# globc/mrAudio

Hardware: AMD Instinct MI355X
Metric: clips/s encode+fuse+score, 32-clip x 32-frame synthetic (higher is better)
Workload: dtype f16

## Files before the change

### include/mra.h

```cpp
#ifndef MRA_H_
#define MRA_H_

#include <stddef.h>
#include <stdint.h>

#ifdef __cplusplus
extern "C" {
#endif

#define MRA_OK 0
#define MRA_EINVAL (-1)
#define MRA_ESTATE (-2)
#define MRA_EHIP (-3)
#define MRA_ENOMEM (-4)
#define MRA_ENAME (-5)

#define MRA_F32 0
#define MRA_F16 1
#define MRA_BF16 2

typedef struct mra_qformer mra_qformer;

typedef struct mra_cfg {
  int32_t hidden;
// ... 230 lines not shown
int mra_debug_self_attention(const void* qkv, const int64_t* mask, int32_t dtype, int32_t items, int32_t S, int32_t heads, void* ctx, float* lse,
                             void* stream);
int mra_debug_ln_rows(const float* x, const int64_t* x_view, int32_t rows, int32_t H, const float* const* params, int32_t lane_rows, int32_t period,
                      int32_t split, float eps, float* y32, const int64_t* y32_view, void* y16, const int64_t* y16_view, int32_t dtype, void* stream);
int mra_debug_embed_ln(const int64_t* ids, int32_t items, int32_t L, int32_t Q, int32_t H, int32_t vocab, const float* query, int64_t query_item_stride,
                       const float* word, const float* pos, const float* gain, const float* bias, float eps, float* h32, void* h16, float* pre32,
                       int32_t dtype, void* stream);
int mra_debug_modality_ln(const void* x, int32_t x_dtype, const int64_t* item_index, int32_t items, int32_t tokens, int32_t E, const float* gain,
                          const float* bias, float eps, void* out, int32_t dtype, void* stream);
int mra_debug_softmax_rows(const float* S, int64_t ld_s, void* P, int64_t ld_p, int32_t rows, int32_t kv, int32_t kvp, float scale, int32_t dtype,
                           void* stream);
int mra_debug_fold_query(const void* x, const int64_t* x_view, size_t x_bytes, const void* w_q, size_t w_q_bytes, const float* b_q, size_t b_q_bytes,
                         const void* w_k, size_t w_k_bytes, void* q_prime, size_t q_prime_bytes, int32_t rows, int32_t H, int32_t E, int32_t Q,
                         int32_t heads, int32_t dtype, void* stream);
int64_t mra_debug_fold_query_launches(void);
int64_t mra_debug_fold_rowfactor_launches(void);
int mra_debug_fold_rowfactor(const float* stat_m, const float* stat_l, float* factors, int32_t rows, int32_t R, int32_t ntiles, void* P, int64_t ld_p,
                             int32_t tile_cols, int32_t kvp, int32_t* hist, void* stream);
int mra_debug_softmax_rescale(void* P, int64_t ld_p, const float* stat_m, const float* stat_l, int32_t rows, int32_t ntiles, int32_t tile_cols,
                              int32_t kvp, int32_t dtype, int32_t* hist, void* stream);
int mra_debug_transpose_pad(const void* src, void* dst, int32_t R, int32_t C, int32_t ld_d, int64_t src_bs, int64_t dst_bs, int32_t batch, int32_t dtype,
                            void* stream);
int mra_debug_split(int32_t kind, const float* src, const int64_t* src_view, int32_t rows, int32_t C, int32_t chunk, int32_t parts, void* dst,
                    int32_t dtype, void* stream);

int mra_debug_gemm_tn_group(int32_t njobs, const void* const* dY, const int64_t* y_views, const int64_t* y_block_stride, const void* const* X,
                            const int64_t* x_views, const int64_t* x_block_stride, float* const* dW, float* const* db, const int32_t* M,
                            const int32_t* N, const int32_t* K, const int32_t* ldw, const int32_t* accumulate, int32_t dtype, void* stream);
int mra_debug_ln_bwd(const void* const* ptrs_a, const int64_t* views_a, int32_t rows_a, float eps_a, const void* const* ptrs_b, const int64_t* views_b,
                     int32_t rows_b, float eps_b, int32_t H, int32_t dtype, void* stream);
// ... 46 lines not shown
```

### mraudio_amd/_lib.py

```python
from __future__ import annotations

import ctypes as C
import os

import torch

MRA_F32, MRA_F16, MRA_BF16 = 0, 1, 2
_ERR = {-1: "MRA_EINVAL", -2: "MRA_ESTATE", -3: "MRA_EHIP", -4: "MRA_ENOMEM", -5: "MRA_ENAME"}

LIB_NAME = "libmra_hip.so"
LIB_PATH = os.path.join(os.path.dirname(os.path.abspath(__file__)), LIB_NAME)


class mra_cfg(C.Structure):
    _fields_ = [
        ("hidden", C.c_int32), ("heads", C.c_int32), ("inter", C.c_int32), ("layers", C.c_int32),
        ("cross_freq", C.c_int32), ("enc_width", C.c_int32), ("n_query", C.c_int32), ("vocab", C.c_int32),
        ("max_pos", C.c_int32), ("ln_eps", C.c_float), ("enc_ln_eps", C.c_float), ("llm_hidden", C.c_int32),
        ("op_dtype", C.c_int32),
    ]


class mra_vit_cfg(C.Structure):
    _fields_ = [("dim", C.c_int32), ("heads", C.c_int32), ("mlp", C.c_int32), ("depth", C.c_int32), ("patch", C.c_int32),
# ... 165 lines not shown
                                          C.c_int32, C.c_int32, C.c_int32, C.c_void_p, C.c_void_p, C.c_void_p, C.c_void_p]),
    "mra_debug_beats_attention": (C.c_int, [C.c_void_p, C.c_int32, C.c_void_p, C.c_void_p, C.c_int32, C.c_int32, C.c_void_p, C.c_void_p]),
    "mra_debug_beats_posconv": (C.c_int, [C.c_void_p, C.c_void_p, C.c_int32, C.c_int32, C.c_void_p]),
    "mra_debug_self_attention": (C.c_int, [C.c_void_p, C.c_void_p, C.c_int32, C.c_int32, C.c_int32, C.c_int32, C.c_void_p, C.c_void_p, C.c_void_p]),
    "mra_debug_ln_rows": (C.c_int, [C.c_void_p, C.POINTER(C.c_int64), C.c_int32, C.c_int32, C.POINTER(C.c_void_p), C.c_int32, C.c_int32, C.c_int32,
                                    C.c_float, C.c_void_p, C.POINTER(C.c_int64), C.c_void_p, C.POINTER(C.c_int64), C.c_int32, C.c_void_p]),
    "mra_debug_embed_ln": (C.c_int, [C.c_void_p, C.c_int32, C.c_int32, C.c_int32, C.c_int32, C.c_int32, C.c_void_p, C.c_int64, C.c_void_p, C.c_void_p,
                                     C.c_void_p, C.c_void_p, C.c_float, C.c_void_p, C.c_void_p, C.c_void_p, C.c_int32, C.c_void_p]),
    "mra_debug_modality_ln": (C.c_int, [C.c_void_p, C.c_int32, C.c_void_p, C.c_int32, C.c_int32, C.c_int32, C.c_void_p, C.c_void_p, C.c_float,
                                        C.c_void_p, C.c_int32, C.c_void_p]),
    "mra_debug_softmax_rows": (C.c_int, [C.c_void_p, C.c_int64, C.c_void_p, C.c_int64, C.c_int32, C.c_int32, C.c_int32, C.c_float, C.c_int32,
                                         C.c_void_p]),
    "mra_debug_fold_query": (C.c_int, [C.c_void_p, C.c_void_p, C.c_size_t, C.c_void_p, C.c_size_t, C.c_void_p, C.c_size_t, C.c_void_p, C.c_size_t,
                                       C.c_void_p, C.c_size_t, C.c_int32, C.c_int32, C.c_int32, C.c_int32, C.c_int32, C.c_int32, C.c_void_p]),
    "mra_debug_fold_query_launches": (C.c_int64, []),
    "mra_debug_fold_rowfactor_launches": (C.c_int64, []),
    "mra_debug_fold_rowfactor": (C.c_int, [C.c_void_p, C.c_void_p, C.c_void_p, C.c_int32, C.c_int32, C.c_int32, C.c_void_p, C.c_int64, C.c_int32,
                                           C.c_int32, C.c_void_p, C.c_void_p]),
    "mra_debug_softmax_rescale": (C.c_int, [C.c_void_p, C.c_int64, C.c_void_p, C.c_void_p, C.c_int32, C.c_int32, C.c_int32, C.c_int32, C.c_int32,
                                            C.c_void_p, C.c_void_p]),
    "mra_debug_transpose_pad": (C.c_int, [C.c_void_p, C.c_void_p, C.c_int32, C.c_int32, C.c_int32, C.c_int64, C.c_int64, C.c_int32, C.c_int32,
                                          C.c_void_p]),
    "mra_debug_split": (C.c_int, [C.c_int32, C.c_void_p, C.POINTER(C.c_int64), C.c_int32, C.c_int32, C.c_int32, C.c_int32, C.c_void_p, C.c_int32,
                                  C.c_void_p]),
    "mra_debug_gemm_tn_group": (C.c_int, [C.c_int32, C.POINTER(C.c_void_p), C.POINTER(C.c_int64), C.POINTER(C.c_int64), C.POINTER(C.c_void_p),
                                          C.POINTER(C.c_int64), C.POINTER(C.c_int64), C.POINTER(C.c_void_p), C.POINTER(C.c_void_p), C.POINTER(C.c_int32),
                                          C.POINTER(C.c_int32), C.POINTER(C.c_int32), C.POINTER(C.c_int32), C.POINTER(C.c_int32), C.c_int32, C.c_void_p]),
    "mra_debug_ln_bwd": (C.c_int, [C.POINTER(C.c_void_p), C.POINTER(C.c_int64), C.c_int32, C.c_float, C.POINTER(C.c_void_p), C.POINTER(C.c_int64),
                                   C.c_int32, C.c_float, C.c_int32, C.c_int32, C.c_void_p]),
    "mra_debug_embed_bwd": (C.c_int, [C.c_void_p, C.c_void_p, C.c_int32, C.c_int32, C.c_int32, C.c_int32, C.c_int32, C.c_void_p, C.c_void_p, C.c_void_p,
# ... 84 lines not shown
```

### mraudio_amd/csrc/attention.hip

```cpp
#include "kernels.h"
#include "mra_common.h"

namespace mra {

namespace {

typedef int i32x4v __attribute__((ext_vector_type(4)));

constexpr int KVT = 32;
constexpr int TILE_B = KVT * 128;
constexpr int WAVE_LDS = 4 * TILE_B;
constexpr int OPAD = 68;
constexpr float LOG2E = 1.4426950408889634f;
constexpr int PART_STRIDE = 32 * 64 + 64;
constexpr int SH_TPS = 2;
constexpr int SH_STAGES = 3;
constexpr int SH_STAGE_B = SH_TPS * 2 * TILE_B;
constexpr int SH_PARK_B = (32 * OPAD + 64) * 4;
constexpr int SH_LDS = SH_STAGES * SH_STAGE_B > 4 * SH_PARK_B ? SH_STAGES * SH_STAGE_B : 4 * SH_PARK_B;

template <typename T, bool MASKED, int SPLITW>
__global__ void __launch_bounds__(256) attn_kernel(const AttnArgs a) {
  extern __shared__ __attribute__((aligned(16))) char smem[];
  const int tid = threadIdx.x;
  const int lane = tid & 63;
  const int wave = __builtin_amdgcn_readfirstlane(tid >> 6);
  const int qblocks = (a.q_rows + 31) >> 5;
  const int nunits = a.items * a.heads * qblocks;
  const int ntiles_all = (a.kv_len + KVT - 1) / KVT;

  int unit, gs;
  if (SPLITW == 1) {
    unit = blockIdx.x * 4 + wave;
    gs = 0;
  } else {
// ... 81 lines not shown
#pragma unroll
  for (int i = 0; i < 16; ++i) { ot[0][i] = 0.f; ot[1][i] = 0.f; }

  const int h4 = 4 * (lane >> 5);
  int buf = 0;
  if (tfirst < te) issue(0, tfirst);
  for (int t = tfirst; t < te; t += tstep) {
    const bool more = t + tstep < te;
    if (more) {
      issue(buf ^ 1, t + tstep);
      asm volatile("s_waitcnt vmcnt(8)" ::: "memory");
    } else {
      asm volatile("s_waitcnt vmcnt(0)" ::: "memory");
    }
    const char* kb = wl + buf * 2 * TILE_B;
    const char* vb = kb + TILE_B;

    f32x16 st;
#pragma unroll
    for (int i = 0; i < 16; ++i) st[i] = 0.f;
#pragma unroll
    for (int s = 0; s < 4; ++s) st = mfma32<T>(lds_read8<T>(kb + koff[s]), qf[s], st);

    const int tok0 = t * KVT;
    float mx = -INFINITY;
#pragma unroll
    for (int g4 = 0; g4 < 4; ++g4) {
      f32x4 madd;
      if (MASKED) {
        madd = *reinterpret_cast<const f32x4*>(wmask + tok0 + 8 * g4 + h4);
      }
#pragma unroll
      for (int e = 0; e < 4; ++e) {
        const int i = 4 * g4 + e;
        float y = st[i] * sl2;
        if (MASKED) {
          y += madd[e];
        } else {
          if (tok0 + 8 * g4 + h4 + e >= a.kv_len) y = -INFINITY;
        }
        st[i] = y;
        mx = fmaxf(mx, y);
      }
    }
    mx = fmaxf(mx, __shfl_xor(mx, 32, 64));
    const float m_new = fmaxf(m_run, mx);
    const float alpha = __builtin_amdgcn_exp2f(m_run - m_new);
    m_run = m_new;
    float psum = 0.f;
#pragma unroll
    for (int i = 0; i < 16; ++i) {
      const float p = __builtin_amdgcn_exp2f(st[i] - m_new);
      st[i] = p;
      psum += p;
    }
    l_run = l_run * alpha + psum;
#pragma unroll
    for (int i = 0; i < 16; ++i) { ot[0][i] *= alpha; ot[1][i] *= alpha; }

    typename Vec8<T>::type pf[2];
#pragma unroll
    for (int s = 0; s < 2; ++s)
#pragma unroll
      for (int j = 0; j < 8; ++j) pf[s][j] = from_f32<T>(st[8 * s + j]);

    {
      const unsigned vaddr0 = wl_lds + buf * 2 * TILE_B + TILE_B + vlane[0];
      const unsigned vaddr1 = wl_lds + buf * 2 * TILE_B + TILE_B + vlane[1];
      i16x4 r00, r01, r02, r03, r10, r11, r12, r13;
      asm volatile(
          "ds_read_b64_tr_b16 %0, %8\n\t"
          "ds_read_b64_tr_b16 %1, %8 offset:1024\n\t"
          "ds_read_b64_tr_b16 %2, %8 offset:2048\n\t"
          "ds_read_b64_tr_b16 %3, %8 offset:3072\n\t"
          "ds_read_b64_tr_b16 %4, %9\n\t"
          "ds_read_b64_tr_b16 %5, %9 offset:1024\n\t"
          "ds_read_b64_tr_b16 %6, %9 offset:2048\n\t"
          "ds_read_b64_tr_b16 %7, %9 offset:3072\n\t"
          "s_waitcnt lgkmcnt(0)"
          : "=&v"(r00), "=&v"(r01), "=&v"(r02), "=&v"(r03), "=&v"(r10), "=&v"(r11), "=&v"(r12), "=&v"(r13)
          : "v"(vaddr0), "v"(vaddr1)
          : "memory");
      auto cat = [](i16x4 lo, i16x4 hi) {
        i16x8 v8;
        v8[0] = lo[0]; v8[1] = lo[1]; v8[2] = lo[2]; v8[3] = lo[3];
        v8[4] = hi[0]; v8[5] = hi[1]; v8[6] = hi[2]; v8[7] = hi[3];
        return __builtin_bit_cast(typename Vec8<T>::type, v8);
      };
      ot[0] = mfma32<T>(cat(r00, r01), pf[0], ot[0]);
      ot[0] = mfma32<T>(cat(r02, r03), pf[1], ot[0]);
      ot[1] = mfma32<T>(cat(r10, r11), pf[0], ot[1]);
      ot[1] = mfma32<T>(cat(r12, r13), pf[1], ot[1]);
    }
    buf ^= 1;
  }

  const float l_tot = l_run + __shfl_xor(l_run, 32, 64);
  float* ow = reinterpret_cast<float*>(wl);
  float* mw = ow + 32 * OPAD;
  float* lw = mw + 32;
  {
    const int q = lane & 31;
#pragma unroll
    for (int mt = 0; mt < 2; ++mt)
#pragma unroll
      for (int g4 = 0; g4 < 4; ++g4) {
        f32x4 v = {ot[mt][4 * g4], ot[mt][4 * g4 + 1], ot[mt][4 * g4 + 2], ot[mt][4 * g4 + 3]};
        *reinterpret_cast<f32x4*>(ow + q * OPAD + 32 * mt + 8 * g4 + h4) = v;
// ... 63 lines not shown
    const f32x4 x1 = *reinterpret_cast<const f32x4*>(ps + q * 64 + 8 * dc + 4);
#pragma unroll
    for (int e = 0; e < 4; ++e) { o[e] += wgt * x0[e]; o[4 + e] += wgt * x1[e]; }
  }
  const int q0 = qb * 32;
  if (q0 + q >= a.q_rows) return;
  if (a.lse && dc == 0) a.lse[((long long)item * a.heads + head) * a.q_rows + q0 + q] = M + __builtin_amdgcn_logf(L);
  const float inv = 1.0f / L;
  typename Vec8<T>::type r;
#pragma unroll
  for (int e = 0; e < 8; ++e) r[e] = from_f32<T>(o[e] * inv);
  T* op = (T*)a.O + (long long)item * a.o_item_stride + (long long)(q0 + q) * a.o_ld + head * 64 + 8 * dc;
  *reinterpret_cast<typename Vec8<T>::type*>(op) = r;
}

template <typename T>
int launch_t(const AttnArgs& a, hipStream_t stream) {
  const int qblocks = (a.q_rows + 31) >> 5;
  const int nunits = a.items * a.heads * qblocks;
  const int ntiles = (a.kv_len + KVT - 1) / KVT;
  const bool masked = a.mask != nullptr;
  const bool shared = ntiles >= 8 && !masked;
  size_t lds = 4 * WAVE_LDS + (masked ? (size_t)4 * ntiles * KVT * sizeof(float) : 0);
  if (lds > 160 * 1024) return -1;
  void (*kfn)(const AttnArgs);
  dim3 grid;
  if (shared) {
    kfn = attn_kernel<T, false, 4>;
    grid = dim3(nunits * a.nsplit);
  } else {
    if (a.nsplit != 1) return -1;
    kfn = masked ? attn_kernel<T, true, 1> : attn_kernel<T, false, 1>;
    grid = dim3((nunits + 3) / 4);
  }
  if (lds > 64 * 1024) {
    if (hipFuncSetAttribute((const void*)kfn, hipFuncAttributeMaxDynamicSharedMemorySize, (int)lds) != hipSuccess)
      return -3;
  }
  hipLaunchKernelGGL(kfn, grid, dim3(256), lds, stream, a);
  if (shared && a.nsplit > 1) {
    hipLaunchKernelGGL(attn_combine_kernel<T>, dim3(nunits), dim3(256), 0, stream, a);
  }
  return hipGetLastError() == hipSuccess ? 0 : -4;
}

template <typename T>
__global__ void __launch_bounds__(256) attn_shared_kernel(const AttnArgs a) {
  extern __shared__ __attribute__((aligned(16))) char smem[];
  const int tid = threadIdx.x;
  const int lane = tid & 63;
  const int wave = __builtin_amdgcn_readfirstlane(tid >> 6);
  const int groups = (a.kv_share + 3) >> 2;
  const int ntiles_all = (a.kv_len + KVT - 1) / KVT;
  const int nstages_all = (ntiles_all + SH_TPS - 1) / SH_TPS;

  int b = blockIdx.x;
  const int gs = b % a.nsplit; b /= a.nsplit;
  const int grp = b % groups; b /= groups;
  const int head = b % a.heads;
// ... 229 lines not shown
    if ((long long)nunits * s >= 1536) break;
  }
  return best;
}

int launch_attention(const AttnArgs& args, int op_dtype, hipStream_t stream) {
  AttnArgs a = args;
  if (a.kv_share < 1) a.kv_share = 1;
  if (a.items <= 0 || a.heads <= 0 || a.q_rows <= 0 || a.kv_len <= 0 || a.nsplit < 1) return -1;
  if (a.nsplit > 1 && !a.part) return -1;
  if ((a.q_ld | a.o_ld | a.k_ld | a.v_ld) & 7) return -1;
  if (a.items % a.kv_share) return -1;
  return op_dtype == OP_F16 ? launch_t<f16>(a, stream) : launch_t<bf16>(a, stream);
}

int attn_shared_pick_split(int kv_items, int kv_share, int heads, int kv_len) {
  const int units = kv_items * heads * ((kv_share + 3) / 4);
  const int ntiles = (kv_len + KVT - 1) / KVT;
  const int nstages = (ntiles + SH_TPS - 1) / SH_TPS;
  if (ntiles < 64) return 1;
  int best = 1;
  for (int s = 1; s <= 16; ++s) {
    if (nstages / s < 8) break;
    best = s;
    if ((long long)units * s >= 512) break;
  }
  return best;
}

int launch_attention_shared(const AttnArgs& args, int op_dtype, hipStream_t stream) {
// ... 10 lines not shown
```

### mraudio_amd/csrc/kernels.h

```cpp
#pragma once
#include <hip/hip_runtime.h>
#include <stdint.h>

namespace mra {

enum OpDtype { OP_F16 = 0, OP_BF16 = 1 };

enum GemmEpi {
  EPI_OP = 0,
  EPI_GELU_OP = 1,
  EPI_RES_F32 = 2,
  EPI_F32 = 3,
  EPI_KV = 4,
  EPI_GELU_BOTH = 6,
  EPI_GELU_BWD = 7,
  EPI_RES_OP = 8,
  EPI_RES_LN = 9,
  EPI_RES_F32_STAT = 10,
  EPI_RES_OP_STAT = 13,
  EPI_LNF_OP = 11,
  EPI_LNF_GELU_OP = 12,
  EPI_SOFTPART = 5,
};

// ... 248 lines not shown
  int k_ld, v_ld;
  const long long* mask;
  int mask_ld;
  int items, heads, q_rows, kv_len;
  float scale;
  int nsplit;
  float* part;
  float* lse;
  int kv_share = 1;
};
size_t attn_partial_bytes(int items, int heads, int q_rows, int nsplit);
int attn_pick_split(int items, int heads, int q_rows, int kv_len);
int launch_attention(const AttnArgs& a, int op_dtype, hipStream_t stream);
int attn_shared_pick_split(int kv_items, int kv_share, int heads, int kv_len);
int launch_attention_shared(const AttnArgs& a, int op_dtype, hipStream_t stream);

int launch_ln_rows(const float* x, RowView xv, int rows, int H, const float* gain, const float* bias, float eps,
                   float* y32, RowView y32v, void* y16, RowView y16v, int op_dtype, hipStream_t stream);
int launch_ln_rows2(const float* x, RowView xv, int rows, int H, const float* gain, const float* bias, const float* gain2,
                    const float* bias2, int period, int split, float eps, float* y32, RowView y32v, void* y16, RowView y16v,
                    int op_dtype, hipStream_t stream);
int launch_ln_rows4(const float* x, RowView xv, int rows, int H, const float* gain, const float* bias, const float* gain2, const float* bias2,
                    int lane_rows, const float* gain3, const float* bias3, const float* gain4, const float* bias4, int period, int split,
                    float eps, float* y32, RowView y32v, void* y16, RowView y16v, int op_dtype, hipStream_t stream);
int launch_modality_ln(const void* x, int x_dtype, const long long* item_index, int items, int tokens, int E,
                       const float* gain, const float* bias, float eps, void* out, int op_dtype, hipStream_t stream);
int launch_embed_ln(const long long* ids, int items, int L, int Q, int H, int vocab, const float* query,
                    long long query_item_stride, const float* word,
                    const float* pos, const float* gain, const float* bias, float eps, float* h32, void* h16,
                    float* pre32 , int op_dtype, hipStream_t stream);
// ... 22 lines not shown
```

### mraudio_amd/csrc/mra_abi.hip

```cpp
#include <cmath>
#include <cstdio>
#include <cstdlib>

#include "mra_handle.h"

using namespace mra;
using namespace mra_host;

namespace mra_host {
thread_local std::string g_err;
}

namespace {

size_t layout_params(mra_qformer* h, char* base) {
  const mra_cfg& c = h->cfg;
  const size_t H = c.hidden, I = c.inter, E = c.enc_width;
  Carver cv(base);
  size_t goff = 0;
  auto reg = [&](const std::string& name, void* p, int dtype, long long numel) {
    Param pr;
    pr.ptr = p;
    pr.dtype = dtype;
    pr.numel = numel;
// ... 580 lines not shown
  return per_item * items;
}

namespace {
int check_loaded(mra_qformer* h) {
  char names[256];
  const int miss = mra_qformer_missing(h, names, sizeof(names));
  int tolerated = 0;
  for (const char* opt : {"ln.weight", "ln.bias", "llm_proj.weight", "llm_proj.bias"}) {
    auto it = h->params.find(opt);
    if (it != h->params.end() && !it->second.loaded) ++tolerated;
  }
  return miss > tolerated ? fail(MRA_ESTATE, std::string("parameters not loaded: ") + names) : MRA_OK;
}

int run_lanes(Lane* lanes, int nl, const int64_t* input_ids, const int64_t* attention_mask, int N, int L, void* workspace, hipStream_t stream) {
  const mra_qformer* h = lanes[0].h;
  const mra_cfg& c = h->cfg;
  const bool pair = nl == 2;
  const int Q = c.n_query, S = Q + L, H = c.hidden, I = c.inter;
  const int op = h->op();
  long long* mask2 = nullptr;
  layout_lanes(lanes, nl, (char*)workspace, N, L, &mask2);
  const Work& w = lanes[0].w;
  const long long SH = (long long)S * H;
  const size_t esz = 2;

  const RowView all_rows = plain(N * S, H), all_lanes = plain(nl * N * S, H);
  const RowView q_view = items_view(SH, Q, H);
  const RowView t_view = items_view(SH, L > 0 ? L : 1, H);
  const RowView cls_view = items_view(SH, 1, H);
  const RowView qc_rows = plain(N * Q, H);
  const size_t t_off16 = (size_t)Q * H * esz;
  const size_t t_off32 = (size_t)Q * H;

  const bool ln_fuse = !pair && (h->chain_ring & 12) == 12 && H % 96 == 0 && H % 256 == 0 && H <= 1024;
  int rc;
  for (int l = 0; l < nl; ++l) {
    Lane& x = lanes[l];
    mra_qformer* hl = x.h;
    rc = launch_embed_ln((const long long*)input_ids, N, L, Q, H, hl->cfg.vocab, x.query, x.query_stride, hl->word, hl->pos, hl->embg, hl->embb,
                         c.ln_eps, x.w.hA32, x.w.hA16, nullptr, op, stream);
    if (rc) return chk(rc, "embed_ln");
    if (ln_fuse) HIP_TRY(hipMemsetAsync(w.lncnt, 0, w.lncnt_bytes, stream));
    if (x.plan.form != CrossPlan::KV_CACHE) {
      if (x.plan.form == CrossPlan::FOLD && !x.plan.kmajor) {
        const int E = hl->cfg.enc_width, kvp = fold_kvp(x.kv);
        rc = launch_transpose_pad(x.enc, x.w.encT, x.kv, E, kvp, (long long)x.kv * E, (long long)E * kvp, N, op, stream);
        if (rc) return chk(rc, "enc transpose");
      }
// ... 9 lines not shown
  }
  const long long* mask = (const long long*)attention_mask;
  if (pair && mask) {
    HIP_TRY(hipMemcpyAsync(mask2, mask, (size_t)N * S * 8, hipMemcpyDeviceToDevice, stream));
    HIP_TRY(hipMemcpyAsync(mask2 + (size_t)N * S, mask, (size_t)N * S * 8, hipMemcpyDeviceToDevice, stream));
    mask = mask2;
  }

  const bool want_text_last = lanes[0].out_full != nullptr;
  bool want_cls_last = false;
  for (int l = 0; l < nl; ++l) want_cls_last |= !want_text_last && lanes[l].out_cls;

  for (int i = 0; i < c.layers; ++i) {
    const LayerW* Lw[2] = {&lanes[0].h->layers[i], &lanes[nl - 1].h->layers[i]};
    const bool last = i == c.layers - 1;
    {
      GemmProb p[2] = {};
      for (int l = 0; l < nl; ++l) {
        p[l].A = lanes[l].w.hA16; p[l].a = all_rows;
        p[l].W = Lw[l]->wqkv; p[l].bias = Lw[l]->bqkv;
        p[l].C = lanes[l].w.qkv16; p[l].c = plain(N * S, 3 * H);
        p[l].M = N * S; p[l].N = 3 * H; p[l].K = H;
        p[l].tile_cfg = N * S >= 1024 ? GT_128 : GT_AUTO;
        if ((lanes[l].h->chain_ring & 1) && N * S >= 1024 && (3 * H) % 144 == 0) p[l].tile_cfg = GT_RING_144x128;
      }
      rc = launch_gemm(p, nl, EPI_OP, op, stream);
      if (rc) return chk(rc, "qkv gemm");
    }
    rc = launch_attention(self_attn_args(c, w.qkv16, w.ctx16, mask, nl * N, S), op, stream);
    if (rc) return chk(rc, "self attention");
    {
      GemmProb p[2] = {};
      for (int l = 0; l < nl; ++l) {
        p[l].A = lanes[l].w.ctx16; p[l].a = all_rows;
        p[l].W = Lw[l]->wo; p[l].bias = Lw[l]->bo;
        p[l].R = lanes[l].w.hA32; p[l].r = all_rows;
        p[l].C = lanes[l].w.pre32; p[l].c = all_rows;
        p[l].M = N * S; p[l].N = H; p[l].K = H;
        if ((lanes[l].h->chain_ring & 4) && N * S >= 1024 && H % 96 == 0) p[l].tile_cfg = GT_RING_96x64;
      }
      if (ln_fuse && p[0].tile_cfg == GT_RING_96x64) {
        p[0].ln_gain = Lw[0]->ln1g; p[0].ln_bias = Lw[0]->ln1b; p[0].ln_eps = c.ln_eps;
        p[0].ln_y32 = w.hB32; p[0].ln_y32v = all_rows; p[0].ln_y16 = w.hB16; p[0].ln_y16v = all_rows; p[0].ln_counter = w.lncnt;
        rc = launch_gemm(p, 1, EPI_RES_LN, op, stream);
        if (rc) return chk(rc, "attn out gemm + ln");
// ... 551 lines not shown
    if (value < 0 || value > 1000) return fail(MRA_EINVAL, "auto_split_pmax_milli is a threshold on p_max in [0, 1000] thousandths");
    h->auto_tau_milli = value;
    return MRA_OK;
  }
  if (key == "chain_ring") {
    if (value < 0 || value > 15) return fail(MRA_EINVAL, "chain_ring is a mask of bits 0-3");
    h->chain_ring = value;
    return MRA_OK;
  }
  if (key == "cross_fuse") {
    if (value < 0 || (value & ~7))
      return fail(MRA_EINVAL, "cross_fuse is a mask of 1 (query projection and Q' in one launch), 2 (row factors inside the P.enc launch) and 4 (context GEMM on the 64 x 64 tile)");
    h->cross_fuse = value;
    return MRA_OK;
  }
  if (key == "multi_core") {
    if (value < 0 || value > 1) return fail(MRA_EINVAL, "multi_core is 0 (attn_kernel with kv_share) or 1 (shared-stream core)");
    h->multi_core = value;
    return MRA_OK;
  }
  return fail(MRA_ENAME, "unknown option: " + key);
}

int mra_qformer_set_kv_done_event(mra_qformer* h, void* ev) {
  if (!h) return fail(MRA_EINVAL, "null handle");
  h->kv_done = reinterpret_cast<hipEvent_t>(ev);
  return MRA_OK;
}

size_t mra_kv_cache_bytes(mra_qformer* h, int32_t items, int32_t kv) {
// ... 789 lines not shown
  if (rows == 0) return MRA_OK;
  if (!x || !w_q || !w_k || !q_prime) return fail(MRA_EINVAL, "null argument");
  if (!dbg_aligned(x, 16) || !dbg_aligned(w_q, 16) || !dbg_aligned(w_k, 16) || !dbg_aligned(q_prime, 16) || !dbg_aligned(b_q, 16))
    return fail(MRA_EINVAL, "misaligned buffer");
  if (!dbg_fits(dbg_extent(xv, rows, H), 2, 0, x_bytes)) return fail(MRA_EINVAL, "x: the view and H leave x_bytes");
  if (!dbg_fits((u128)heads * 64 * (u128)H, 2, 0, w_q_bytes)) return fail(MRA_EINVAL, "w_q: heads * 64 rows of H leave w_q_bytes");
  if (b_q && !dbg_fits((u128)heads * 64, 4, 0, b_q_bytes)) return fail(MRA_EINVAL, "b_q: heads * 64 floats leave b_q_bytes");
  if (!dbg_fits((u128)heads * (u128)E * 64, 2, 0, w_k_bytes)) return fail(MRA_EINVAL, "w_k: heads blocks of [E][64] leave w_k_bytes");
  if (!dbg_fits((u128)rows * (u128)heads * (u128)E, 2, 0, q_prime_bytes)) return fail(MRA_EINVAL, "q_prime: rows * heads * E elements leave q_prime_bytes");
  return chk(launch_fold_query(x, xv, w_q, b_q, w_k, q_prime, rows, H, E, Q, heads, op, as_stream(stream)), "fold_query");
}

int64_t mra_debug_fold_query_launches(void) { return fold_query_launch_count(); }
int64_t mra_debug_fold_rowfactor_launches(void) { return fold_rowfactor_launch_count(); }

}
```

### mraudio_amd/csrc/mra_handle.h

```cpp
#pragma once
#include <hip/hip_runtime.h>

#include <algorithm>
#include <cstdlib>
#include <cstring>
#include <map>
#include <string>
#include <vector>

#include "../../include/mra.h"
#include "kernels.h"
#include "mra_common.h"

namespace mra_host {

using namespace mra;

extern thread_local std::string g_err;

inline int fail(int code, const std::string& msg) {
  g_err = msg;
  return code;
}

// ... 105 lines not shown
  float *encg = nullptr, *encb = nullptr;
  void* wkv = nullptr;
  float* bkv = nullptr;
  void* wllm = nullptr;
  float* bllm = nullptr;
  char* arena_f = nullptr;
  bool fold_stale = true;
  bool raw_features = true;
  bool inreg_rescale = true;
  int fold_tile = mra::GT_128;
  bool fold_stream = false;
  int cross_mode = 0;
  int chain_ring = 7;
  int train_ring = 4;
  int cross_fuse = 1;
  int multi_core = 1;
  int cross_precise = 0;
  float* wk32 = nullptr;
  char* arena_p = nullptr;
  bool precise_stale = true;
  bool cross_auto = false;
  bool auto_stale = true;
  int auto_resolved = -1;
  int auto_probes = 0;
  int auto_tau_milli = 500;
  int* auto_hist = nullptr;
  int* auto_hist_host = nullptr;
  std::vector<float> auto_median;
  hipEvent_t kv_done = nullptr;
  hipEvent_t kv_ev0 = nullptr, kv_ev1 = nullptr;
// ... 54 lines not shown
```

Measured before the change: 4942.

## Fuse QKV projection GEMM and self-attention into one kernel launch

```diff
diff --git a/include/mra.h b/include/mra.h
--- a/include/mra.h
+++ b/include/mra.h
@@ -268,6 +268,12 @@
                          const void* w_k, size_t w_k_bytes, void* q_prime, size_t q_prime_bytes, int32_t rows, int32_t H, int32_t E, int32_t Q,
                          int32_t heads, int32_t dtype, void* stream);
 int64_t mra_debug_fold_query_launches(void);
+int mra_debug_qkv_attention(const void* rows, const void* wqkv, const float* bqkv, const int64_t* mask, int32_t dtype, int32_t items, int32_t S,
+                            int32_t heads, void* ctx, void* stream);
+int64_t mra_debug_qkv_attention_launches(void);
+int64_t mra_debug_attention_launches(int32_t masked);
+int32_t mra_debug_self_fuse_plan(int32_t option, int32_t chain_ring, int32_t lanes, int32_t items, int32_t S, int32_t hidden, int32_t heads,
+                                 int32_t dtype, int32_t want_full);
 int64_t mra_debug_fold_rowfactor_launches(void);
 int mra_debug_fold_rowfactor(const float* stat_m, const float* stat_l, float* factors, int32_t rows, int32_t R, int32_t ntiles, void* P, int64_t ld_p,
                              int32_t tile_cols, int32_t kvp, int32_t* hist, void* stream);
diff --git a/mraudio_amd/_lib.py b/mraudio_amd/_lib.py
--- a/mraudio_amd/_lib.py
+++ b/mraudio_amd/_lib.py
@@ -203,6 +203,11 @@
     "mra_debug_fold_query": (C.c_int, [C.c_void_p, C.c_void_p, C.c_size_t, C.c_void_p, C.c_size_t, C.c_void_p, C.c_size_t, C.c_void_p, C.c_size_t,
                                        C.c_void_p, C.c_size_t, C.c_int32, C.c_int32, C.c_int32, C.c_int32, C.c_int32, C.c_int32, C.c_void_p]),
     "mra_debug_fold_query_launches": (C.c_int64, []),
+    "mra_debug_qkv_attention": (C.c_int, [C.c_void_p, C.c_void_p, C.c_void_p, C.c_void_p, C.c_int32, C.c_int32, C.c_int32, C.c_int32, C.c_void_p,
+                                          C.c_void_p]),
+    "mra_debug_qkv_attention_launches": (C.c_int64, []),
+    "mra_debug_attention_launches": (C.c_int64, [C.c_int32]),
+    "mra_debug_self_fuse_plan": (C.c_int32, [C.c_int32, C.c_int32, C.c_int32, C.c_int32, C.c_int32, C.c_int32, C.c_int32, C.c_int32, C.c_int32]),
     "mra_debug_fold_rowfactor_launches": (C.c_int64, []),
     "mra_debug_fold_rowfactor": (C.c_int, [C.c_void_p, C.c_void_p, C.c_void_p, C.c_int32, C.c_int32, C.c_int32, C.c_void_p, C.c_int64, C.c_int32,
                                            C.c_int32, C.c_void_p, C.c_void_p]),
diff --git a/mraudio_amd/csrc/attention.hip b/mraudio_amd/csrc/attention.hip
--- a/mraudio_amd/csrc/attention.hip
+++ b/mraudio_amd/csrc/attention.hip
@@ -1,3 +1,6 @@
+#include <atomic>
+#include <type_traits>
+
 #include "kernels.h"
 #include "mra_common.h"
 
@@ -19,6 +22,87 @@
 constexpr int SH_PARK_B = (32 * OPAD + 64) * 4;
 constexpr int SH_LDS = SH_STAGES * SH_STAGE_B > 4 * SH_PARK_B ? SH_STAGES * SH_STAGE_B : 4 * SH_PARK_B;
 
+template <typename T, bool MASKED>
+__device__ __forceinline__ void attn_tile_step(const char* kb, unsigned vtile, const int (&koff)[4], const unsigned (&vlane)[2],
+                                               const typename Vec8<T>::type (&qf)[4], const float* wm, int tok0, int kv_len, float sl2, int h4,
+                                               float& m_run, float& l_run, f32x16 (&ot)[2]) {
+  f32x16 st;
+#pragma unroll
+  for (int i = 0; i < 16; ++i) st[i] = 0.f;
+#pragma unroll
+  for (int s = 0; s < 4; ++s) st = mfma32<T>(lds_read8<T>(kb + koff[s]), qf[s], st);
+
+  float mx = -INFINITY;
+#pragma unroll
+  for (int g4 = 0; g4 < 4; ++g4) {
+    f32x4 madd;
+    if (MASKED) {
+      madd = *reinterpret_cast<const f32x4*>(wm + 8 * g4 + h4);
+    }
+#pragma unroll
+    for (int e = 0; e < 4; ++e) {
+      const int i = 4 * g4 + e;
+      float y = st[i] * sl2;
+      if (MASKED) {
+        y += madd[e];
+      } else {
+        if (tok0 + 8 * g4 + h4 + e >= kv_len) y = -INFINITY;
+      }
+      st[i] = y;
+      mx = fmaxf(mx, y);
+    }
+  }
+  mx = fmaxf(mx, __shfl_xor(mx, 32, 64));
+  const float m_new = fmaxf(m_run, mx);
+  const float alpha = __builtin_amdgcn_exp2f(m_run - m_new);
+  m_run = m_new;
+  float psum = 0.f;
+#pragma unroll
+  for (int i = 0; i < 16; ++i) {
+    const float p = __builtin_amdgcn_exp2f(st[i] - m_new);
+    st[i] = p;
+    psum += p;
+  }
+  l_run = l_run * alpha + psum;
+#pragma unroll
+  for (int i = 0; i < 16; ++i) { ot[0][i] *= alpha; ot[1][i] *= alpha; }
+
+  typename Vec8<T>::type pf[2];
+#pragma unroll
+  for (int s = 0; s < 2; ++s)
+#pragma unroll
+    for (int j = 0; j < 8; ++j) pf[s][j] = from_f32<T>(st[8 * s + j]);
+
+  {
+    const unsigned vaddr0 = vtile + vlane[0];
+    const unsigned vaddr1 = vtile + vlane[1];
+    i16x4 r00, r01, r02, r03, r10, r11, r12, r13;
+    asm volatile(
+        "ds_read_b64_tr_b16 %0, %8\n\t"
+        "ds_read_b64_tr_b16 %1, %8 offset:1024\n\t"
+        "ds_read_b64_tr_b16 %2, %8 offset:2048\n\t"
+        "ds_read_b64_tr_b16 %3, %8 offset:3072\n\t"
+        "ds_read_b64_tr_b16 %4, %9\n\t"
+        "ds_read_b64_tr_b16 %5, %9 offset:1024\n\t"
+        "ds_read_b64_tr_b16 %6, %9 offset:2048\n\t"
+        "ds_read_b64_tr_b16 %7, %9 offset:3072\n\t"
+        "s_waitcnt lgkmcnt(0)"
+        : "=&v"(r00), "=&v"(r01), "=&v"(r02), "=&v"(r03), "=&v"(r10), "=&v"(r11), "=&v"(r12), "=&v"(r13)
+        : "v"(vaddr0), "v"(vaddr1)
+        : "memory");
+    auto cat = [](i16x4 lo, i16x4 hi) {
+      i16x8 v8;
+      v8[0] = lo[0]; v8[1] = lo[1]; v8[2] = lo[2]; v8[3] = lo[3];
+      v8[4] = hi[0]; v8[5] = hi[1]; v8[6] = hi[2]; v8[7] = hi[3];
+      return __builtin_bit_cast(typename Vec8<T>::type, v8);
+    };
+    ot[0] = mfma32<T>(cat(r00, r01), pf[0], ot[0]);
+    ot[0] = mfma32<T>(cat(r02, r03), pf[1], ot[0]);
+    ot[1] = mfma32<T>(cat(r10, r11), pf[0], ot[1]);
+    ot[1] = mfma32<T>(cat(r12, r13), pf[1], ot[1]);
+  }
+}
+
 template <typename T, bool MASKED, int SPLITW>
 __global__ void __launch_bounds__(256) attn_kernel(const AttnArgs a) {
   extern __shared__ __attribute__((aligned(16))) char smem[];
@@ -130,84 +214,8 @@
       asm volatile("s_waitcnt vmcnt(0)" ::: "memory");
     }
     const char* kb = wl + buf * 2 * TILE_B;
-    const char* vb = kb + TILE_B;
-
-    f32x16 st;
-#pragma unroll
-    for (int i = 0; i < 16; ++i) st[i] = 0.f;
-#pragma unroll
-    for (int s = 0; s < 4; ++s) st = mfma32<T>(lds_read8<T>(kb + koff[s]), qf[s], st);
-
-    const int tok0 = t * KVT;
-    float mx = -INFINITY;
-#pragma unroll
-    for (int g4 = 0; g4 < 4; ++g4) {
-      f32x4 madd;
-      if (MASKED) {
-        madd = *reinterpret_cast<const f32x4*>(wmask + tok0 + 8 * g4 + h4);
-      }
-#pragma unroll
-      for (int e = 0; e < 4; ++e) {
-        const int i = 4 * g4 + e;
-        float y = st[i] * sl2;
-        if (MASKED) {
-          y += madd[e];
-        } else {
-          if (tok0 + 8 * g4 + h4 + e >= a.kv_len) y = -INFINITY;
-        }
-        st[i] = y;
-        mx = fmaxf(mx, y);
-      }
-    }
-    mx = fmaxf(mx, __shfl_xor(mx, 32, 64));
-    const float m_new = fmaxf(m_run, mx);
-    const float alpha = __builtin_amdgcn_exp2f(m_run - m_new);
-    m_run = m_new;
-    float psum = 0.f;
-#pragma unroll
-    for (int i = 0; i < 16; ++i) {
-      const float p = __builtin_amdgcn_exp2f(st[i] - m_new);
-      st[i] = p;
-      psum += p;
-    }
-    l_run = l_run * alpha + psum;
-#pragma unroll
-    for (int i = 0; i < 16; ++i) { ot[0][i] *= alpha; ot[1][i] *= alpha; }
-
-    typename Vec8<T>::type pf[2];
-#pragma unroll
-    for (int s = 0; s < 2; ++s)
-#pragma unroll
-      for (int j = 0; j < 8; ++j) pf[s][j] = from_f32<T>(st[8 * s + j]);
-
-    {
-      const unsigned vaddr0 = wl_lds + buf * 2 * TILE_B + TILE_B + vlane[0];
-      const unsigned vaddr1 = wl_lds + buf * 2 * TILE_B + TILE_B + vlane[1];
-      i16x4 r00, r01, r02, r03, r10, r11, r12, r13;
-      asm volatile(
-          "ds_read_b64_tr_b16 %0, %8\n\t"
-          "ds_read_b64_tr_b16 %1, %8 offset:1024\n\t"
-          "ds_read_b64_tr_b16 %2, %8 offset:2048\n\t"
-          "ds_read_b64_tr_b16 %3, %8 offset:3072\n\t"
-          "ds_read_b64_tr_b16 %4, %9\n\t"
-          "ds_read_b64_tr_b16 %5, %9 offset:1024\n\t"
-          "ds_read_b64_tr_b16 %6, %9 offset:2048\n\t"
-          "ds_read_b64_tr_b16 %7, %9 offset:3072\n\t"
-          "s_waitcnt lgkmcnt(0)"
-          : "=&v"(r00), "=&v"(r01), "=&v"(r02), "=&v"(r03), "=&v"(r10), "=&v"(r11), "=&v"(r12), "=&v"(r13)
-          : "v"(vaddr0), "v"(vaddr1)
-          : "memory");
-      auto cat = [](i16x4 lo, i16x4 hi) {
-        i16x8 v8;
-        v8[0] = lo[0]; v8[1] = lo[1]; v8[2] = lo[2]; v8[3] = lo[3];
-        v8[4] = hi[0]; v8[5] = hi[1]; v8[6] = hi[2]; v8[7] = hi[3];
-        return __builtin_bit_cast(typename Vec8<T>::type, v8);
-      };
-      ot[0] = mfma32<T>(cat(r00, r01), pf[0], ot[0]);
-      ot[0] = mfma32<T>(cat(r02, r03), pf[1], ot[0]);
-      ot[1] = mfma32<T>(cat(r10, r11), pf[0], ot[1]);
-      ot[1] = mfma32<T>(cat(r12, r13), pf[1], ot[1]);
-    }
+    attn_tile_step<T, MASKED>(kb, wl_lds + buf * 2 * TILE_B + TILE_B, koff, vlane, qf, MASKED ? wmask + t * KVT : nullptr, t * KVT, a.kv_len, sl2, h4,
+                              m_run, l_run, ot);
     buf ^= 1;
   }
 
@@ -301,6 +309,8 @@
   *reinterpret_cast<typename Vec8<T>::type*>(op) = r;
 }
 
+std::atomic<long long>& attn_launch_counter(bool masked);
+
 template <typename T>
 int launch_t(const AttnArgs& a, hipStream_t stream) {
   const int qblocks = (a.q_rows + 31) >> 5;
@@ -328,8 +338,262 @@
   if (shared && a.nsplit > 1) {
     hipLaunchKernelGGL(attn_combine_kernel<T>, dim3(nunits), dim3(256), 0, stream, a);
   }
-  return hipGetLastError() == hipSuccess ? 0 : -4;
-}
+  if (hipGetLastError() != hipSuccess) return -4;
+  if (!shared) attn_launch_counter(masked).fetch_add(1, std::memory_order_relaxed);
+  return 0;
+}
+
+struct QkvAttnArgs {
+  const void* X;
+  const void* W;
+  const float* bias;
+  const long long* mask;
+  void* O;
+  int N, S, H, heads;
+  float scale;
+};
+
+template <typename T>
+__global__ void __launch_bounds__(512) qkv_attn_kernel(const QkvAttnArgs a) {
+  constexpr int BK = 64, ROWB = BK * 2, G = 2;
+  constexpr int TN = 192, TM = 64 * G, WGN = 2, WGM = 2, STAGES = 4;
+  constexpr int NWC = WGN * WGM, NW = 2 * NWC;
+  constexpr int WTN = TN / WGN, WTM = TM / WGM, FN = WTN / 16, FM = WTM / 16;
+  constexpr int ROWS = TN + TM, NPIECE = ROWS / 8, PPW = NPIECE / NW;
+  constexpr int BUF = ROWS * ROWB;
+  constexpr int RED_BYTES = NWC * FN * FM * 1024;
+  constexpr int HEAD_B = 64 * ROWB, SLOT_B = 3 * HEAD_B;
+  constexpr int PRIV_B = 16384, PRIV_MASK = 32 * OPAD * 4 + 256;
+  static_assert(NPIECE == PPW * NW && (STAGES - 3) * PPW <= 63, "every wave stages PPW whole pieces per K tile; vmcnt holds 6 bits");
+  static_assert(RED_BYTES + G * SLOT_B <= STAGES * BUF && (FN * FM) % 2 == 0, "exchange area + Q/K/V tiles reuse the ring");
+  static_assert(4 * PRIV_B <= RED_BYTES && PRIV_MASK + 64 * 4 <= PRIV_B && WTM == 64, "phase 2 scratch lies in the exchange area");
+  extern __shared__ __attribute__((aligned(16))) char smem[];
+  using V8 = typename Vec8<T>::type;
+  const int tid = threadIdx.x;
+  const int lane = tid & 63;
+  const int wave = __builtin_amdgcn_readfirstlane(tid >> 6);
+  const int group = wave / NWC, gw = wave - group * NWC;
+  const int wn0 = (gw / WGM) * WTN;
+  const int wm0 = (gw % WGM) * WTM;
+  const int head = blockIdx.x % a.heads, item0 = (blockIdx.x / a.heads) * G;
+  const int S = a.S, H = a.H, N = a.N;
+  const int nk = H / BK;
+
+  const char* src[PPW];
+#pragma unroll
+  for (int i = 0; i < PPW; ++i) {
+    const int p = wave + i * NW;
+    const int row = p * 8 + (lane >> 3), c = (lane & 7) ^ ((row >> 1) & 7);
+    if (row < TN) {
+      const long long wr = (long long)(row >> 6) * H + head * 64 + (row & 63);
+      src[i] = (const char*)a.W + (wr * H + c * 8) * 2;
+    } else {
+      const int m = row - TN;
+      const int item = min(item0 + (m >> 6), N - 1), tok = min(m & 63, S - 1);
+      src[i] = (const char*)a.X + (((long long)item * S + tok) * H + c * 8) * 2;
+    }
+  }
+  auto stage = [&](int slot, int kt) {
+    char* base = smem + slot * BUF + wave * 1024;
+    const long long koff = (long long)kt * ROWB;
+#pragma unroll
+    for (int i = 0; i < PPW; ++i) glds16(src[i] + koff, base + i * (NW * 1024));
+  };
+#pragma unroll
+  for (int t = 0; t < STAGES - 2; ++t)
+    if (t < nk) stage(t, t);
+  int foff[2];
+#pragma unroll
+  for (int ks = 0; ks < 2; ++ks) {
+    const int r = lane & 15;
+    const int c = (4 * ks + (lane >> 4)) ^ ((r >> 1) & 7);
+    foff[ks] = r * ROWB + c * 16;
+  }
+  f32x4 acc[FN][FM];
+#pragma unroll
+  for (int i = 0; i < FN; ++i)
+#pragma unroll
+    for (int j = 0; j < FM; ++j) acc[i][j] = f32x4{0.f, 0.f, 0.f, 0.f};
+
+  {
+    V8 fa[2][FN], fb[2][FM];
+    int rslot = 0, fslot = STAGES - 2;
+    auto interval = [&](auto GRP, auto PAR, int kt) {
+      constexpr int g = decltype(GRP)::value, par = decltype(PAR)::value;
+      if (kt < nk) {
+        if (kt + STAGES - 3 < nk) asm volatile("s_waitcnt vmcnt(%0)" ::"n"((STAGES - 3) * PPW) : "memory");
+        else asm volatile("s_waitcnt vmcnt(0)" ::: "memory");
+      }
+      asm volatile("" ::: "memory");
+      __builtin_amdgcn_s_barrier();
+      asm volatile("" ::: "memory");
+      if constexpr (par == g) {
+        if (kt < nk) {
+          const char* wb = smem + rslot * BUF + wn0 * ROWB;
+          const char* xb = smem + rslot * BUF + TN * ROWB + wm0 * ROWB;
+#pragma unroll
+          for (int ks = 0; ks < 2; ++ks) {
+#pragma unroll
+            for (int i = 0; i < FN; ++i) fa[ks][i] = lds_read8<T>(wb + i * 16 * ROWB + foff[ks]);
+#pragma unroll
+            for (int j = 0; j < FM; ++j) fb[ks][j] = lds_read8<T>(xb + j * 16 * ROWB + foff[ks]);
+          }
+        }
+      } else {
+        if (kt >= 1) {
+          __builtin_amdgcn_s_setprio(1);
+#pragma unroll
+          for (int ks = 0; ks < 2; ++ks)
+#pragma unroll
+            for (int i = 0; i < FN; ++i)
+#pragma unroll
+              for (int j = 0; j < FM; ++j) acc[i][j] = mfma16<T>(fa[ks][i], fb[ks][j], acc[i][j]);
+          __builtin_amdgcn_s_setprio(0);
+        }
+      }
+      if (kt + STAGES - 2 < nk) stage(fslot, kt + STAGES - 2);
+      rslot = rslot + 1 == STAGES ? 0 : rslot + 1;
+      fslot = fslot + 1 == STAGES ? 0 : fslot + 1;
+    };
+    auto run = [&](auto GRP) {
+#pragma clang loop unroll(disable)
+      for (int kt = 0; kt <= nk; kt += 2) {
+        interval(GRP, std::integral_constant<int, 0>{}, kt);
+        if (kt + 1 <= nk) interval(GRP, std::integral_constant<int, 1>{}, kt + 1);
+      }
+    };
+    if (group == 0) run(std::integral_constant<int, 0>{}); else run(std::integral_constant<int, 1>{});
+  }
+
+  f32x4 bvs[FN];
+  {
+    const int ln = (lane >> 4) * 4;
+#pragma unroll
+    for (int i = 0; i < FN; ++i) {
+      const int n = wn0 + i * 16 + ln;
+      bvs[i] = f32x4{0.f, 0.f, 0.f, 0.f};
+      if (a.bias) bvs[i] = *reinterpret_cast<const f32x4*>(a.bias + (long long)(n >> 6) * H + head * 64 + (n & 63));
+    }
+  }
+  __syncthreads();
+  char* const qkv = smem + RED_BYTES;
+  {
+    constexpr int HALF = FN * FM / 2;
+    f32x4* out_red = reinterpret_cast<f32x4*>(smem) + ((size_t)(group * NWC + gw) * HALF) * 64 + lane;
+    const f32x4* in_red = reinterpret_cast<const f32x4*>(smem) + ((size_t)((group ^ 1) * NWC + gw) * HALF) * 64 + lane;
+#pragma unroll
+    for (int i = 0; i < FN; ++i)
+#pragma unroll
+      for (int j = 0; j < FM; ++j)
+        if (((i * FM + j) & 1) != group) out_red[((i * FM + j) >> 1) * 64] = acc[i][j];
+    __syncthreads();
+    const int lm = lane & 15, ln = (lane >> 4) * 4;
+    char* const slot_base = qkv + (wm0 >> 6) * SLOT_B;
+#pragma unroll
+    for (int i = 0; i < FN; ++i) {
+      const int n = wn0 + i * 16 + ln, blk = n >> 6, d = n & 63;
+      const f32x4 bv = bvs[i];
+#pragma unroll
+      for (int j = 0; j < FM; ++j) {
+        if (((i * FM + j) & 1) != group) continue;
+        const f32x4 v = acc[i][j] + in_red[((i * FM + j) >> 1) * 64] + bv;
+        typename Vec4<T>::type o;
+#pragma unroll
+        for (int e = 0; e < 4; ++e) o[e] = from_f32<T>(v[e]);
+        const int tok = j * 16 + lm;
+        const int swz = blk == 2 ? ((tok >> 1) & 1) << 2 : (tok >> 1) & 7;
+        *reinterpret_cast<typename Vec4<T>::type*>(slot_base + blk * HEAD_B + tok * ROWB + (((d >> 3) ^ swz) << 4) + (d & 4) * 2) = o;
+      }
+    }
+  }
+  __syncthreads();
+
+  const int qblocks = (S + 31) >> 5;
+  if (wave >= G * qblocks) return;
+  const int slot = wave / qblocks, qb = wave - slot * qblocks;
+  const int item = item0 + slot;
+  if (item >= N) return;
+  const int q0 = qb * 32;
+  char* const priv = smem + wave * PRIV_B;
+  float* const wmask = reinterpret_cast<float*>(priv + PRIV_MASK);
+  {
+    float v = -INFINITY;
+    if (lane < S) {
+      const long long mv = a.mask ? a.mask[(long long)item * S + lane] : 1;
+      v = (1.0f - (float)mv) * (-10000.0f * LOG2E);
+    }
+    wmask[lane] = v;
+  }
+  const char* const qt = qkv + slot * SLOT_B;
+  int koff[4];
+  {
+    const int r = lane & 31, h = lane >> 5;
+#pragma unroll
+    for (int s = 0; s < 4; ++s) koff[s] = r * 128 + (((2 * s + h) ^ ((r >> 1) & 7)) << 4);
+  }
+  unsigned vlane[2];
+  {
+    const int g = lane >> 4, i = lane & 15, q4 = i >> 2, p = i & 3, h = lane >> 5;
+    const int row = 4 * h + q4;
+#pragma unroll
+    for (int mt = 0; mt < 2; ++mt) {
+      const int c = 4 * mt + 2 * (g & 1) + (p >> 1);
+      const int pc = c ^ (((q4 >> 1) & 1) << 2);
+      vlane[mt] = row * 128 + pc * 16 + (p & 1) * 8;
+    }
+  }
+  V8 qf[4];
+#pragma unroll
+  for (int s = 0; s < 4; ++s) qf[s] = lds_read8<T>(qt + q0 * ROWB + koff[s]);
+  const unsigned v_lds = (unsigned)(size_t)(__attribute__((address_space(3))) char*)(qt + 2 * HEAD_B);
+  const float sl2 = a.scale * LOG2E;
+  float m_run = -1e30f, l_run = 0.f;
+  f32x16 ot[2];
+#pragma unroll
+  for (int i = 0; i < 16; ++i) { ot[0][i] = 0.f; ot[1][i] = 0.f; }
+  const int h4 = 4 * (lane >> 5);
+  asm volatile("s_waitcnt lgkmcnt(0)" ::: "memory");
+  for (int t = 0; t < qblocks; ++t)
+    attn_tile_step<T, true>(qt + HEAD_B + t * TILE_B, v_lds + t * TILE_B, koff, vlane, qf, wmask + t * KVT, t * KVT, S, sl2, h4, m_run, l_run, ot);
+
+  const float l_tot = l_run + __shfl_xor(l_run, 32, 64);
+  float* ow = reinterpret_cast<float*>(priv);
+  float* mw = ow + 32 * OPAD;
+  float* lw = mw + 32;
+  {
+    const int q = lane & 31;
+#pragma unroll
+    for (int mt = 0; mt < 2; ++mt)
+#pragma unroll
+      for (int g4 = 0; g4 < 4; ++g4) {
+        f32x4 v = {ot[mt][4 * g4], ot[mt][4 * g4 + 1], ot[mt][4 * g4 + 2], ot[mt][4 * g4 + 3]};
+        *reinterpret_cast<f32x4*>(ow + q * OPAD + 32 * mt + 8 * g4 + h4) = v;
+      }
+    if (lane < 32) { mw[q] = m_run; lw[q] = l_tot; }
+  }
+  asm volatile("s_waitcnt lgkmcnt(0)" ::: "memory");
+  for (int idx = lane; idx < 256; idx += 64) {
+    const int q = idx >> 3, dc = idx & 7;
+    const float M = fmaxf(-1e30f, mw[q]);
+    const float wgt = __builtin_amdgcn_exp2f(mw[q] - M);
+    const float L = 0.f + wgt * lw[q];
+    const f32x4 x0 = *reinterpret_cast<const f32x4*>(ow + q * OPAD + 8 * dc);
+    const f32x4 x1 = *reinterpret_cast<const f32x4*>(ow + q * OPAD + 8 * dc + 4);
+    float o[8];
+#pragma unroll
+    for (int e = 0; e < 4; ++e) { o[e] = 0.f + wgt * x0[e]; o[4 + e] = 0.f + wgt * x1[e]; }
+    if (q0 + q >= S) continue;
+    const float inv = 1.0f / L;
+    V8 r;
+#pragma unroll
+    for (int e = 0; e < 8; ++e) r[e] = from_f32<T>(o[e] * inv);
+    T* op = (T*)a.O + ((long long)item * S + q0 + q) * H + head * 64 + 8 * dc;
+    *reinterpret_cast<V8*>(op) = r;
+  }
+}
+
+std::atomic<long long> g_qkv_attn_launches, g_attn_launches[2];
+std::atomic<long long>& attn_launch_counter(bool masked) { return g_attn_launches[masked ? 1 : 0]; }
 
 template <typename T>
 __global__ void __launch_bounds__(256) attn_shared_kernel(const AttnArgs a) {
@@ -589,6 +853,28 @@
   return op_dtype == OP_F16 ? launch_t<f16>(a, stream) : launch_t<bf16>(a, stream);
 }
 
+bool qkv_attn_supported(int S, int H, int heads) { return S >= 1 && S <= 64 && heads >= 1 && H == heads * 64; }
+
+int launch_qkv_attention(const void* X, const void* wqkv, const float* bqkv, const long long* mask, void* ctx, int N, int S, int H, int heads,
+                         int op_dtype, hipStream_t stream) {
+  if (N <= 0) return 0;
+  if (!X || !wqkv || !ctx || !qkv_attn_supported(S, H, heads) || (op_dtype != OP_F16 && op_dtype != OP_BF16)) return -1;
+  const long long groups = ((long long)N + 1) / 2;
+  if (groups * heads > 0x7fffffffLL) return -1;
+  const QkvAttnArgs a{X, wqkv, bqkv, mask, ctx, N, S, H, heads, 0.125f};
+  constexpr size_t lds = 4 * (192 + 128) * 128;
+  const void* fn = op_dtype == OP_F16 ? (const void*)qkv_attn_kernel<f16> : (const void*)qkv_attn_kernel<bf16>;
+  if (!ensure_lds(fn, lds)) return -3;
+  const dim3 grid((unsigned)(groups * heads));
+  if (op_dtype == OP_F16) hipLaunchKernelGGL(qkv_attn_kernel<f16>, grid, dim3(512), lds, stream, a);
+  else hipLaunchKernelGGL(qkv_attn_kernel<bf16>, grid, dim3(512), lds, stream, a);
+  if (hipGetLastError() != hipSuccess) return -4;
+  g_qkv_attn_launches.fetch_add(1, std::memory_order_relaxed);
+  return 0;
+}
+long long qkv_attn_launch_count() { return g_qkv_attn_launches.load(std::memory_order_relaxed); }
+long long attn_launch_count(int masked) { return g_attn_launches[masked ? 1 : 0].load(std::memory_order_relaxed); }
+
 int attn_shared_pick_split(int kv_items, int kv_share, int heads, int kv_len) {
   const int units = kv_items * heads * ((kv_share + 3) / 4);
   const int ntiles = (kv_len + KVT - 1) / KVT;
diff --git a/mraudio_amd/csrc/kernels.h b/mraudio_amd/csrc/kernels.h
--- a/mraudio_amd/csrc/kernels.h
+++ b/mraudio_amd/csrc/kernels.h
@@ -286,6 +286,11 @@
 int launch_attention(const AttnArgs& a, int op_dtype, hipStream_t stream);
 int attn_shared_pick_split(int kv_items, int kv_share, int heads, int kv_len);
 int launch_attention_shared(const AttnArgs& a, int op_dtype, hipStream_t stream);
+bool qkv_attn_supported(int S, int H, int heads);
+int launch_qkv_attention(const void* X, const void* wqkv, const float* bqkv, const long long* mask, void* ctx, int N, int S, int H, int heads,
+                         int op_dtype, hipStream_t stream);
+long long qkv_attn_launch_count();
+long long attn_launch_count(int masked);
 
 int launch_ln_rows(const float* x, RowView xv, int rows, int H, const float* gain, const float* bias, float eps,
                    float* y32, RowView y32v, void* y16, RowView y16v, int op_dtype, hipStream_t stream);
diff --git a/mraudio_amd/csrc/mra_abi.hip b/mraudio_amd/csrc/mra_abi.hip
--- a/mraudio_amd/csrc/mra_abi.hip
+++ b/mraudio_amd/csrc/mra_abi.hip
@@ -618,6 +618,11 @@
   return miss > tolerated ? fail(MRA_ESTATE, std::string("parameters not loaded: ") + names) : MRA_OK;
 }
 
+bool self_fuse_plan(int option, int lanes, long long rows, int S, int hidden, int heads, int op, int chain_ring, bool want_full) {
+  return option == 1 && lanes == 1 && !want_full && (op == OP_F16 || op == OP_BF16) && qkv_attn_supported(S, hidden, heads) && (chain_ring & 1) && rows >= 1024 &&
+         (3 * hidden) % 144 == 0;
+}
+
 int run_lanes(Lane* lanes, int nl, const int64_t* input_ids, const int64_t* attention_mask, int N, int L, void* workspace, hipStream_t stream) {
   const mra_qformer* h = lanes[0].h;
   const mra_cfg& c = h->cfg;
@@ -638,6 +643,7 @@
   const size_t t_off16 = (size_t)Q * H * esz;
   const size_t t_off32 = (size_t)Q * H;
 
+  const bool self_fuse = self_fuse_plan(h->self_fuse, nl, (long long)N * S, S, H, c.heads, op, h->chain_ring, lanes[0].out_full != nullptr);
   const bool ln_fuse = !pair && (h->chain_ring & 12) == 12 && H % 96 == 0 && H % 256 == 0 && H <= 1024;
   int rc;
   for (int l = 0; l < nl; ++l) {
@@ -677,21 +683,26 @@
   for (int i = 0; i < c.layers; ++i) {
     const LayerW* Lw[2] = {&lanes[0].h->layers[i], &lanes[nl - 1].h->layers[i]};
     const bool last = i == c.layers - 1;
-    {
-      GemmProb p[2] = {};
-      for (int l = 0; l < nl; ++l) {
-        p[l].A = lanes[l].w.hA16; p[l].a = all_rows;
-        p[l].W = Lw[l]->wqkv; p[l].bias = Lw[l]->bqkv;
-        p[l].C = lanes[l].w.qkv16; p[l].c = plain(N * S, 3 * H);
-        p[l].M = N * S; p[l].N = 3 * H; p[l].K = H;
-        p[l].tile_cfg = N * S >= 1024 ? GT_128 : GT_AUTO;
-        if ((lanes[l].h->chain_ring & 1) && N * S >= 1024 && (3 * H) % 144 == 0) p[l].tile_cfg = GT_RING_144x128;
+    if (self_fuse) {
+      rc = launch_qkv_attention(w.hA16, Lw[0]->wqkv, Lw[0]->bqkv, mask, w.ctx16, N, S, H, c.heads, op, stream);
+      if (rc) return chk(rc, "qkv + self attention");
+    } else {
+      {
+        GemmProb p[2] = {};
+        for (int l = 0; l < nl; ++l) {
+          p[l].A = lanes[l].w.hA16; p[l].a = all_rows;
+          p[l].W = Lw[l]->wqkv; p[l].bias = Lw[l]->bqkv;
+          p[l].C = lanes[l].w.qkv16; p[l].c = plain(N * S, 3 * H);
+          p[l].M = N * S; p[l].N = 3 * H; p[l].K = H;
+          p[l].tile_cfg = N * S >= 1024 ? GT_128 : GT_AUTO;
+          if ((lanes[l].h->chain_ring & 1) && N * S >= 1024 && (3 * H) % 144 == 0) p[l].tile_cfg = GT_RING_144x128;
+        }
+        rc = launch_gemm(p, nl, EPI_OP, op, stream);
+        if (rc) return chk(rc, "qkv gemm");
       }
-      rc = launch_gemm(p, nl, EPI_OP, op, stream);
-      if (rc) return chk(rc, "qkv gemm");
+      rc = launch_attention(self_attn_args(c, w.qkv16, w.ctx16, mask, nl * N, S), op, stream);
+      if (rc) return chk(rc, "self attention");
     }
-    rc = launch_attention(self_attn_args(c, w.qkv16, w.ctx16, mask, nl * N, S), op, stream);
-    if (rc) return chk(rc, "self attention");
     {
       GemmProb p[2] = {};
       for (int l = 0; l < nl; ++l) {
@@ -1273,6 +1284,11 @@
     h->cross_fuse = value;
     return MRA_OK;
   }
+  if (key == "self_fuse") {
+    if (value < 0 || value > 1) return fail(MRA_EINVAL, "self_fuse is 0 (QKV GEMM, then the self-attention core) or 1 (both in one launch)");
+    h->self_fuse = value;
+    return MRA_OK;
+  }
   if (key == "multi_core") {
     if (value < 0 || value > 1) return fail(MRA_EINVAL, "multi_core is 0 (attn_kernel with kv_share) or 1 (shared-stream core)");
     h->multi_core = value;
@@ -2092,4 +2108,25 @@
 int64_t mra_debug_fold_query_launches(void) { return fold_query_launch_count(); }
 int64_t mra_debug_fold_rowfactor_launches(void) { return fold_rowfactor_launch_count(); }
 
-}
+int mra_debug_qkv_attention(const void* rows, const void* wqkv, const float* bqkv, const int64_t* mask, int32_t dtype, int32_t items, int32_t S,
+                            int32_t heads, void* ctx, void* stream) {
+  int op;
+  if (items < 0 || S < 1 || heads < 1 || heads > 16) return fail(MRA_EINVAL, "sizes: items >= 0, S >= 1, heads in 1..16");
+  if (!dbg_op(dtype, &op)) return fail(MRA_EINVAL, "dtype must be f16 or bf16");
+  if (!qkv_attn_supported(S, heads * 64, heads)) return fail(MRA_EINVAL, "the fused launch takes S <= 64 (longer prompts run the two launches)");
+  if (items == 0) return MRA_OK;
+  if (!rows || !wqkv || !ctx) return fail(MRA_EINVAL, "null argument");
+  if (!dbg_aligned(rows, 16) || !dbg_aligned(wqkv, 16) || !dbg_aligned(ctx, 16) || !dbg_aligned(bqkv, 16))
+    return fail(MRA_EINVAL, "rows, wqkv, bqkv and ctx must be 16-byte aligned");
+  return chk(launch_qkv_attention(rows, wqkv, bqkv, (const long long*)mask, ctx, items, S, heads * 64, heads, op, as_stream(stream)), "qkv + self attention");
+}
+int64_t mra_debug_qkv_attention_launches(void) { return qkv_attn_launch_count(); }
+int64_t mra_debug_attention_launches(int32_t masked) { return attn_launch_count(masked); }
+int32_t mra_debug_self_fuse_plan(int32_t option, int32_t chain_ring, int32_t lanes, int32_t items, int32_t S, int32_t hidden, int32_t heads,
+                                 int32_t dtype, int32_t want_full) {
+  int op;
+  if (!dbg_op(dtype, &op) || items < 0 || S < 0) return 0;
+  return self_fuse_plan(option, lanes, (long long)items * S, S, hidden, heads, op, chain_ring, want_full != 0) ? 1 : 0;
+}
+
+}
diff --git a/mraudio_amd/csrc/mra_handle.h b/mraudio_amd/csrc/mra_handle.h
--- a/mraudio_amd/csrc/mra_handle.h
+++ b/mraudio_amd/csrc/mra_handle.h
@@ -143,6 +143,7 @@
   int chain_ring = 7;
   int train_ring = 4;
   int cross_fuse = 1;
+  int self_fuse = 1;
   int multi_core = 1;
   int cross_precise = 0;
   float* wk32 = nullptr;
```

Measured after the change: 5005, median of 6. +1.3%, better.
